# kmacrow/Shellac

Measured on AMD Instinct MI355X. Metric: cache_ops_per_s, higher is better.
Workload: dtype uint8

## Files before the change

### shellac_amd/csrc/bind.cc

```cpp
#include <pybind11/pybind11.h>
#include <pybind11/stl.h>

#include <hip/hip_runtime_api.h>

#include "bind_parts.h"
#include "hbm_cache.h"
#include "host_cache.h"
#include "trace.h"

namespace py = pybind11;
using namespace shellac;

namespace {

template <typename T>
T* P(uintptr_t p) { return reinterpret_cast<T*>(p); }
hipStream_t S(uintptr_t s) { return reinterpret_cast<hipStream_t>(s); }

py::dict counters_dict(const CacheCounters& c) {
  py::dict d;
  d["get_ops"] = c.get_ops;
  d["get_hits"] = c.get_hits;
  d["get_bytes"] = c.get_bytes;
  d["set_ops"] = c.set_ops;
// ... 93 lines not shown
         py::arg("now"), py::arg("stream"), py::arg("done_slot") = -1)
      .def("serve_get", [](HbmCache& c, uintptr_t host_keys, int64_t n, uintptr_t out,
                           uint64_t out_cap, uintptr_t off, uint32_t now, int done_slot,
                           uintptr_t stream) {
        py::gil_scoped_release nogil;
        return c.serve_get_after(S(stream), P<const Digest>(host_keys), n, P<uint8_t>(out),
                                 out_cap, P<uint64_t>(off), now, done_slot);
      }, py::arg("host_keys"), py::arg("n"), py::arg("out"), py::arg("out_cap"), py::arg("off"),
         py::arg("now"), py::arg("done_slot"), py::arg("stream") = 0)
      .def("serve_wait", [](HbmCache& c, int slot, int64_t timeout_ms) {
        py::gil_scoped_release nogil;
        return c.serve_wait(slot, timeout_ms);
      }, py::arg("slot"), py::arg("timeout_ms") = 10000)
      .def("serve_kick", [](HbmCache& c) {
        py::gil_scoped_release nogil;
        c.serve_kick();
      })
      .def("serve_stop", [](HbmCache& c) {
        py::gil_scoped_release nogil;
        c.serve_stop();
      })
      .def("serve_trace", &HbmCache::serve_trace)
      .def_property_readonly("wall_khz", &HbmCache::wall_khz)
      .def_property_readonly("serve_launches", &HbmCache::serve_launches)
      .def_property_readonly("serve_jobs", &HbmCache::serve_jobs)
      .def("host_slot", &HbmCache::host_slot)
      .def("wait_host_slot", [](const HbmCache& c, int i, int64_t timeout_ms) {
        py::gil_scoped_release nogil;
        return c.wait_host_slot(i, timeout_ms);
      }, py::arg("slot"), py::arg("timeout_ms") = 10000)
      .def("gather", [](HbmCache& c, uintptr_t loc, uintptr_t off, int64_t n, uintptr_t out,
                        uintptr_t s, uint64_t out_cap, uintptr_t first, uintptr_t size,
                        uintptr_t out_size, uintptr_t out_off, uintptr_t table, uintptr_t cslot,
                        uintptr_t prefix, int shift) {
        py::gil_scoped_release nogil;
        c.gather(P<const uint64_t>(loc), P<const uint64_t>(off), n, P<uint8_t>(out), S(s),
                 out_cap, P<const uint32_t>(first), P<const uint64_t>(size), P<uint64_t>(out_size),
                 P<uint64_t>(out_off), P<uint32_t>(table), P<const uint32_t>(cslot),
                 P<const uint64_t>(prefix), shift);
      }, py::arg("loc"), py::arg("off"), py::arg("n"), py::arg("out"), py::arg("stream"),
         py::arg("out_cap") = ~0ull, py::arg("first") = 0, py::arg("size") = 0,
         py::arg("out_size") = 0, py::arg("out_off") = 0, py::arg("table") = 0,
         py::arg("cslot") = 0, py::arg("prefix") = 0, py::arg("shift") = 0)
      .def("store_graph", [](HbmCache& c, HbmCache::StoreGraph& g, uintptr_t keys,
                             uintptr_t values, uintptr_t val_off, uintptr_t vlen, uintptr_t flags,
                             uintptr_t expire, int64_t n, uint64_t bytes_bound, uint32_t now,
                             uintptr_t s) {
        py::gil_scoped_release nogil;
        c.store_graph(&g, P<const Digest>(keys), P<const uint8_t>(values),
                      P<const uint64_t>(val_off), P<const uint32_t>(vlen),
                      P<const uint32_t>(flags), P<const uint32_t>(expire), n, bytes_bound, now,
                      S(s));
      })
      .def("store", [](HbmCache& c, uintptr_t keys, uintptr_t values, uintptr_t val_off,
                       uintptr_t vlen, uintptr_t flags, uintptr_t expire, int64_t n,
                       uint64_t bytes_bound, uint32_t now, uintptr_t s, uintptr_t index_after,
                       uintptr_t append_after, uintptr_t append_done, int phase,
                       uintptr_t plan_done, uintptr_t done) {
        py::gil_scoped_release nogil;
        c.store(P<const Digest>(keys), P<const uint8_t>(values), P<const uint64_t>(val_off),
                P<const uint32_t>(vlen), P<const uint32_t>(flags), P<const uint32_t>(expire), n,
                bytes_bound, now, S(s), reinterpret_cast<hipEvent_t>(index_after), true,
                reinterpret_cast<hipEvent_t>(append_after),
                reinterpret_cast<hipEvent_t>(append_done), phase,
                reinterpret_cast<hipEvent_t>(plan_done), reinterpret_cast<hipEvent_t>(done));
      }, py::arg("keys"), py::arg("values"), py::arg("val_off"), py::arg("vlen"),
         py::arg("flags"), py::arg("expire"), py::arg("n"), py::arg("bytes_bound"), py::arg("now"),
         py::arg("stream"), py::arg("index_after") = 0, py::arg("append_after") = 0,
         py::arg("append_done") = 0, py::arg("phase") = 0, py::arg("plan_done") = 0,
         py::arg("done") = 0)
      .def("remove", [](HbmCache& c, uintptr_t keys, int64_t n, uintptr_t found, uint32_t now,
                        uintptr_t s) {
        py::gil_scoped_release nogil;
        c.remove(P<const Digest>(keys), n, P<uint8_t>(found), now, S(s));
      })
      .def("sweep", [](HbmCache& c, uint32_t now, uintptr_t s) {
// ... 239 lines not shown
```

### shellac_amd/csrc/hbm_cache.h

```cpp
#pragma once

#include <hip/hip_runtime_api.h>

#include <algorithm>
#include <mutex>
#include <string>
#include <vector>

#include "layout.h"

namespace shellac {

enum : int { kEvictFifo = 0, kEvictClock = 1 };

struct ShardConfig {
  uint64_t log_bytes = 1ull << 30;
  uint64_t nbuckets = 1ull << 20;
  uint32_t max_item = 1u << 20;
  int device = 0;
  int evict = kEvictClock;
  uint64_t reinsert_max = 0;
  int serve_blocks = 8;
};

// ... 23 lines not shown
  static constexpr uint64_t kSlotFailed = ~0ull - 1;
  static constexpr int64_t kLookupPrefixWords = 2049;
  void small_get(const Digest* keys, int64_t n, uint8_t* out, uint64_t out_cap, uint64_t* off,
                 uint32_t now, hipStream_t s, int done_slot = -1);
  static constexpr int64_t kSmallGetMax = 1 << 17;
  static constexpr int kServeKeys = 29;
  static constexpr int kServeRing = 16;
  bool serve_get(const Digest* host_keys, int64_t n, uint8_t* out, uint64_t out_cap,
                 uint64_t* off, uint32_t now, int done_slot);
  bool serve_get_after(hipStream_t after, const Digest* host_keys, int64_t n, uint8_t* out,
                       uint64_t out_cap, uint64_t* off, uint32_t now, int done_slot);
  void serve_kick();
  uint64_t serve_backlog() const {
    uint64_t c = 0;
    for (int b = 0; b < srv_blocks_; ++b)
      c += __atomic_load_n(srv_ctl_ + kSrvCtlConsumed + 8 * b, __ATOMIC_ACQUIRE);
    const uint64_t t = __atomic_load_n(&srv_ticket_, __ATOMIC_RELAXED);
    return t > c ? t - c : 0;
  }
  static constexpr int kServeBlocksMax = 8;
  static constexpr int kSrvCtlConsumed = 24;
  int serve_blocks() const { return srv_blocks_; }
  uint64_t serve_wait(int done_slot, int64_t timeout_ms = 10000);
  void serve_stop();
  uint64_t serve_launches() const { return srv_launches_; }
  uint64_t serve_jobs() const { return __atomic_load_n(&srv_ticket_, __ATOMIC_RELAXED); }
  std::vector<uint64_t> serve_trace() const;
  uint64_t wall_khz() const { return srv_khz_; }
  void gather(const uint64_t* loc, const uint64_t* off, int64_t n, uint8_t* out, hipStream_t s,
              uint64_t out_cap = ~0ull, const uint32_t* first = nullptr,
              const uint64_t* size = nullptr, uint64_t* out_size = nullptr,
              uint64_t* out_off = nullptr, uint32_t* table = nullptr,
              const uint32_t* cslot = nullptr, const uint64_t* prefix = nullptr,
              int shift = 0);
  void store(const Digest* keys, const uint8_t* values, const uint64_t* val_off,
             const uint32_t* vlen, const uint32_t* flags, const uint32_t* expire, int64_t n,
             uint64_t bytes_bound, uint32_t now, hipStream_t s, hipEvent_t index_after = nullptr,
             bool allow_reclaim = true, hipEvent_t append_after = nullptr,
             hipEvent_t append_done = nullptr, int phase = 0, hipEvent_t plan_done = nullptr,
             hipEvent_t done = nullptr);
  bool would_reclaim(uint64_t bytes_bound) const {
    return cfg_.evict == kEvictClock && rmax_ && should_reclaim(bytes_bound);
  }
  struct StoreGraph {
    hipGraphExec_t exec[2] = {nullptr, nullptr};
    const void* ptrs[6] = {};
    int64_t n = -1;
    uint64_t bound = 0;
    uint32_t now = 0;
    uint64_t ws_gen = 0;
    uint64_t captures = 0, launches = 0;
  };
  void store_graph(StoreGraph* g, const Digest* keys, const uint8_t* values,
                   const uint64_t* val_off, const uint32_t* vlen, const uint32_t* flags,
                   const uint32_t* expire, int64_t n, uint64_t bytes_bound, uint32_t now,
                   hipStream_t s);
  static void destroy_graph(StoreGraph* g);
  void remove(const Digest* keys, int64_t n, uint8_t* found, uint32_t now, hipStream_t s);
  void sweep(uint32_t now, hipStream_t s, uint64_t* live_entries, uint64_t* live_bytes);
  uint64_t export_keys(Digest* out, uint64_t out_cap, uint32_t now, hipStream_t s);
  void save(const std::string& path, const uint64_t user[4], hipStream_t s);
  void load(const std::string& path, uint64_t user[4], hipStream_t s);
  void flush(hipStream_t s);
  std::vector<uint64_t> debug_bucket(uint64_t b);
  std::vector<uint64_t> debug_hand();
  void debug_set_entry(uint64_t b, int slot, uint64_t d0, uint64_t d1, uint64_t loc,
                       uint32_t vlen, uint32_t expire);
// ... 188 lines not shown
```

### shellac_amd/csrc/hbm_cache.hip

```cpp
#include <hip/hip_runtime.h>
#include <hip/hip_ext.h>
#include <hipcub/hipcub.hpp>

#include <algorithm>
#include <chrono>
#include <cstdlib>
#include <cstring>
#include <type_traits>
#include <vector>

#include "hbm_cache.h"
#include "trace.h"

namespace shellac {

#define HIP_OK(expr)                                                                   \
  do {                                                                                 \
    hipError_t _e = (expr);                                                            \
    if (_e != hipSuccess)                                                              \
      throw Error(std::string("HIP error ") + hipGetErrorString(_e) + " at " + #expr + \
                  " [" + __FILE__ + ":" + std::to_string(__LINE__) + "]");             \
  } while (0)

namespace {
// ... 364 lines not shown
        int he;
        uint64_t hb = bucket1(d, mask);
        group_match(vb[p], d, l8, head, cap, now, &hl, &hv, &he);
        if (hl == 0) {
          hb = bucket2(d, mask);
          const uint4 v2 = reinterpret_cast<const uint4*>(index + hb * kEntriesPerBucket)[l8];
          group_match(v2, d, l8, head, cap, now, &hl, &hv, &he);
        }
        if (l8 == 0) {
          ++ops;
          if (hl) {
            mark_ref(index, hb, he, hv);
            hv = entry_vlen(hv);
            out_loc[i] = (hl - 1) % cap;
            out_size[i] = item_bytes(hv);
            ++hits;
            bytes += hv;
            psum += item_bytes(hv);
          } else {
            out_loc[i] = kMissLoc;
            out_size[i] = 0;
          }
        }
      }
    }
    __syncthreads();
  }
  block_count(ctr, ops, &CacheCounters::get_ops, hits, &CacheCounters::get_hits, bytes,
              &CacheCounters::get_bytes);
  block_partial(psum, part);
}

constexpr int kCoPer = 4;
constexpr int kCoKeys = kBlock * kCoPer;
constexpr int kCoSlots = 2 * kCoKeys;

template <bool PROBE>
__global__ __launch_bounds__(kBlock) __attribute__((amdgpu_waves_per_eu(4))) void k_coalesce(
    const Digest* __restrict__ keys, int64_t n, int64_t plen, uint32_t* __restrict__ tab,
    uint32_t tmask, uint32_t* __restrict__ first, uint32_t* __restrict__ cslot,
    Entry* __restrict__ index, uint64_t mask, const uint64_t* __restrict__ head_ptr,
    uint64_t reserve, uint64_t cap, uint32_t now, uint64_t* __restrict__ out_loc,
    uint64_t* __restrict__ out_size, CacheCounters* __restrict__ ctr,
    uint64_t* __restrict__ part, int local_only, uint64_t* __restrict__ woff) {
  __shared__ Digest s_k[kCoKeys];
  __shared__ unsigned long long s_wt[kBlock / 64], s_run;
  if (threadIdx.x == 0) s_run = 0;
  __shared__ uint32_t s_tab[kCoSlots];
  __shared__ uint32_t s_rep[kCoKeys];
  __shared__ uint32_t s_dup[kCoKeys];
  __shared__ uint32_t s_q[PROBE ? kCoKeys : 1];
  __shared__ int s_qn;
  const uint64_t head = PROBE ? *head_ptr + reserve : 0;
  const int l8 = threadIdx.x & 7;
  unsigned long long ops = 0, hits = 0, bytes = 0, psum = 0, dups = 0;
  const int64_t r0 = (int64_t)blockIdx.x * plen, r1 = min(n, r0 + plen);
  for (int64_t base = r0; base < r1; base += kCoKeys) {
    const int cnt = (int)min((int64_t)kCoKeys, r1 - base);
    for (int k = threadIdx.x; k < kCoSlots; k += kBlock) s_tab[k] = 0;
    for (int k = threadIdx.x; k < kCoKeys; k += kBlock) s_dup[k] = 0;
    if (threadIdx.x == 0) s_qn = 0;
    Digest dk[kCoPer];
    uint32_t lrep[kCoPer];
#pragma unroll
    for (int u = 0; u < kCoPer; ++u) {
      const int j = u * kBlock + threadIdx.x;
      lrep[u] = (uint32_t)j;
      if (j < cnt) {
        dk[u] = keys[base + j];
        s_k[j] = dk[u];
      }
    }
    __syncthreads();
#pragma unroll
    for (int u = 0; u < kCoPer; ++u) {
      const int j = u * kBlock + threadIdx.x;
      if (j >= cnt) continue;
// ... 68 lines not shown
    if (PROBE) {
      const int qn = s_qn;
      constexpr int kG = kBlock / 8;
      for (int q0 = threadIdx.x >> 3; q0 < qn; q0 += kG * kCoProbe) {
        uint4 vb[kCoProbe];
#pragma unroll
        for (int p = 0; p < kCoProbe; ++p) {
          const int q = q0 + p * kG;
          if (q < qn)
            vb[p] = reinterpret_cast<const uint4*>(
                index + bucket1(s_k[s_q[q]], mask) * kEntriesPerBucket)[l8];
        }
#pragma unroll
        for (int p = 0; p < kCoProbe; ++p) {
          const int q = q0 + p * kG;
          if (q >= qn) continue;
          const int j = (int)s_q[q];
          const Digest d = s_k[j];
          uint64_t hl;
          uint32_t hv;
          int he;
          uint64_t hb = bucket1(d, mask);
          group_match(vb[p], d, l8, head, cap, now, &hl, &hv, &he);
          if (hl == 0) {
            hb = bucket2(d, mask);
            const uint4 v2 = reinterpret_cast<const uint4*>(index + hb * kEntriesPerBucket)[l8];
            group_match(v2, d, l8, head, cap, now, &hl, &hv, &he);
          }
          if (l8 == 0) {
            if (hl) mark_ref(index, hb, he, hv);
            hv = entry_vlen(hv);
            ++ops;
            out_loc[base + j] = hl ? (hl - 1) % cap : kMissLoc;
            out_size[base + j] = hl ? item_bytes(hv) : 0;
            if (woff) s_tab[j] = hl ? (uint32_t)item_bytes(hv) : 0u;
            if (hl) {
              ++hits;
              bytes += hv;
              psum += item_bytes(hv);
            }
          }
        }
      }
    }
#pragma unroll
    for (int u = 0; u < kCoPer; ++u) {
      const int j = u * kBlock + threadIdx.x;
      if (j >= cnt) continue;
      const uint32_t f = s_rep[lrep[u]];
      first[base + j] = f;
      if (PROBE && f != (uint32_t)(base + j)) {
        out_loc[base + j] = kMissLoc;
        out_size[base + j] = 0;
        if (woff) s_tab[j] = 0u;
        ++dups;
      }
    }
    __syncthreads();
    if (PROBE && woff) {
      const int t4 = threadIdx.x * kCoPer;
      uint32_t v[kCoPer];
      unsigned long long ts = 0;
#pragma unroll
      for (int u = 0; u < kCoPer; ++u) {
        v[u] = t4 + u < cnt ? s_tab[t4 + u] : 0u;
        ts += v[u];
      }
      const int lane = threadIdx.x & 63, wv = threadIdx.x >> 6;
      unsigned long long inc = ts;
#pragma unroll
      for (int d = 1; d < 64; d <<= 1) {
        const unsigned long long o = __shfl_up(inc, d);
        if (lane >= d) inc += o;
      }
      if (lane == 63) s_wt[wv] = inc;
      __syncthreads();
      unsigned long long ex = s_run + inc - ts, tot = 0;
#pragma unroll
      for (int k = 0; k < kBlock / 64; ++k) {
        if (k < wv) ex += s_wt[k];
        tot += s_wt[k];
      }
#pragma unroll
      for (int u = 0; u < kCoPer; ++u) {
        if (t4 + u < cnt) woff[base + t4 + u] = ex;
        ex += v[u];
      }
      __syncthreads();
      if (threadIdx.x == 0) s_run += tot;
    }
  }
  if (PROBE) {
    if (blockIdx.x == 0 && threadIdx.x == 0) out_size[n] = 0;
    block_count(ctr, ops, &CacheCounters::get_ops, hits, &CacheCounters::get_hits, bytes,
                &CacheCounters::get_bytes);
    block_count(ctr, dups, &CacheCounters::get_coalesced);
    block_partial(psum, part);
  }
}

static_assert(HbmCache::kLookupPrefixWords == kMaxGrid + 1, "prefix words: kMaxGrid + 1");
__global__ __launch_bounds__(kBlock) void k_block_prefix(const uint64_t* __restrict__ part,
                                                         int nparts,
                                                         uint64_t* __restrict__ prefix,
                                                         uint64_t* __restrict__ host_total) {
  constexpr int kPer = kMaxGrid / kBlock;
  __shared__ unsigned long long s_w[kBlock / 64];
  const int lane = threadIdx.x & 63, w = threadIdx.x >> 6;
  uint64_t v[kPer];
  unsigned long long ts = 0;
#pragma unroll
  for (int u = 0; u < kPer; ++u) {
    const int i = threadIdx.x * kPer + u;
    v[u] = i < nparts ? part[i] : 0;
    ts += v[u];
  }
  unsigned long long inc = ts;
#pragma unroll
  for (int d = 1; d < 64; d <<= 1) {
    const unsigned long long o = __shfl_up(inc, d);
    if (lane >= d) inc += o;
  }
  if (lane == 63) s_w[w] = inc;
  __syncthreads();
  unsigned long long ex = inc - ts;
  for (int k = 0; k < w; ++k) ex += s_w[k];
// ... 33 lines not shown
                                                       const uint32_t* __restrict__ cslot) {
  for (int64_t i = (int64_t)blockIdx.x * kBlock + threadIdx.x; i < n;
       i += (int64_t)gridDim.x * kBlock) {
    const uint32_t f = first[i];
    out_size[i] = size[f];
    out_off[i] = off[f];
    if (f == (uint32_t)i && tab) tab[cslot[i]] = 0u;
  }
}

template <typename T>
__device__ __forceinline__ int64_t seg_search(const T* off, int64_t lo, int64_t hi, uint64_t x) {
  while (hi - lo > 1) {
    const int64_t mid = (lo + hi) >> 1;
    if ((uint64_t)off[mid] <= x) lo = mid; else hi = mid;
  }
  return lo;
}

__device__ __forceinline__ int64_t seg_search_global(const uint64_t* off, int64_t n, uint64_t x) {
  int64_t lo = 0, hi = n;
  while (hi - lo > 1) {
    const int64_t mid = (lo + hi) >> 1;
    if (off[mid] <= x) lo = mid; else hi = mid;
  }
  return lo;
}

struct PlainOff {
  const uint64_t* __restrict__ p;
  __device__ __forceinline__ uint64_t operator[](int64_t j) const { return p[j]; }
};
struct BlockedOff {
  const uint64_t* __restrict__ local;
  const uint64_t* __restrict__ prefix;
  int64_t n;
  int shift;
  __device__ __forceinline__ uint64_t operator[](int64_t j) const {
    return j < n ? prefix[j >> shift] + local[j] : prefix[((n - 1) >> shift) + 1];
  }
};

template <typename Off>
__device__ __forceinline__ void block_find2(const Off off, int64_t n1,
                                            uint64_t x0, uint64_t x1, int64_t* s_lo,
                                            int64_t* s_hi, int* s_cnt) {
  const int h = threadIdx.x >> 7, t = threadIdx.x & 127, w = threadIdx.x >> 6;
  const uint64_t x = h ? x1 : x0;
  if (threadIdx.x < 2) {
    s_lo[threadIdx.x] = 0;
    s_hi[threadIdx.x] = n1;
  }
  __syncthreads();
  for (int round = 0; round < 16; ++round) {
    const int64_t lo = s_lo[h], hi = s_hi[h];
    const bool done = (s_hi[0] - s_lo[0] <= 1) && (s_hi[1] - s_lo[1] <= 1);
    if (done) break;
    const int64_t len = hi - lo;
    bool ok = false;
    if (len > 1 && t < 127) {
      const int64_t p = lo + (len * (t + 1) + 127) / 128;
      ok = p < hi && off[p] <= x;
    }
    const unsigned long long b = __ballot(ok);
    __syncthreads();
    if ((threadIdx.x & 63) == 0) s_cnt[w] = __popcll(b);
    __syncthreads();
    if (t == 0 && len > 1) {
      const int k = s_cnt[2 * h] + s_cnt[2 * h + 1];
      const int64_t nlo = k > 0 ? lo + (len * k + 127) / 128 : lo;
      const int64_t nhi = k < 127 ? lo + (len * (k + 1) + 127) / 128 : hi;
      s_lo[h] = nlo;
// ... 27 lines not shown
    if (threadIdx.x < kBlock - 1) {
      const int64_t q = l + (len * (threadIdx.x + 1) + kBlock - 1) / kBlock;
      ok = q < h && off[q] <= x;
    }
    const unsigned long long b = __ballot(ok);
    __syncthreads();
    if ((threadIdx.x & 63) == 0) s_cnt[threadIdx.x >> 6] = __popcll(b);
    __syncthreads();
    if (threadIdx.x == 0) {
      int k = 0;
#pragma unroll
      for (int w = 0; w < kBlock / 64; ++w) k += s_cnt[w];
      const int64_t nlo = k > 0 ? l + (len * k + kBlock - 1) / kBlock : l;
      const int64_t nhi = k < kBlock - 1 ? l + (len * (k + 1) + kBlock - 1) / kBlock : h;
      s_b[0] = nlo;
      s_b[1] = nhi < h ? nhi : h;
    }
    __syncthreads();
  }
  return s_b[0];
}

struct ExpandTail {
  const uint32_t* first = nullptr;
  int64_t n = 0;
  const uint64_t* size = nullptr;
  const uint64_t* off = nullptr;
  uint64_t* out_size = nullptr;
  uint64_t* out_off = nullptr;
  uint32_t* tab = nullptr;
  const uint32_t* cslot = nullptr;
  const uint64_t* prefix = nullptr;
  int shift = 0;
};
__device__ __forceinline__ void expand_tail(const ExpandTail& ex) {
  for (int64_t i = (int64_t)blockIdx.x * kBlock + threadIdx.x; i < ex.n;
       i += (int64_t)gridDim.x * kBlock) {
    const uint32_t f = ex.first[i];
    ex.out_size[i] = ex.size[f];
    ex.out_off[i] = ex.prefix ? ex.prefix[f >> ex.shift] + ex.off[f] : ex.off[f];
    if (f == (uint32_t)i && ex.tab) ex.tab[ex.cslot[i]] = 0u;
  }
}

template <int MODE, int U, int WAVES, bool NTSTORE = false, bool GLDS = false>
__global__ __launch_bounds__(kBlock) __attribute__((amdgpu_waves_per_eu(WAVES))) void k_segcopy(
    const uint8_t* __restrict__ src, const uint64_t* __restrict__ src_off,
    const uint64_t* __restrict__ dst_off, int64_t n, uint8_t* __restrict__ dst,
    const Digest* __restrict__ keys, const uint32_t* __restrict__ vlen,
    const uint32_t* __restrict__ flags, const uint32_t* __restrict__ expire,
    const uint64_t* __restrict__ head_ptr, uint64_t cap, int min_tile, ExpandTail ex) {
  do {
  constexpr int TSC = MODE == 2 ? 768 : GLDS ? 512 : kTileSegCap;
  __shared__ uint64_t s_off[TSC + 1];
  __shared__ __attribute__((aligned(16))) uint8_t s_stage[GLDS ? kBlock / 64 : 1][GLDS ? U : 1]
                                                         [GLDS ? 1024 : 16];
  __shared__ uint64_t s_src[TSC];
  __shared__ int64_t s_lo[2], s_hi[2];
  __shared__ int s_cnt[kBlock / 64];
  if (MODE == 3) n = *reinterpret_cast<const int64_t*>(head_ptr);
  using Off = typename std::conditional<MODE == 4, BlockedOff, PlainOff>::type;
  Off doff;
  if constexpr (MODE == 4)
    doff = BlockedOff{dst_off, ex.prefix, n, ex.shift};
  else
    doff = PlainOff{dst_off};
  const uint64_t total = doff[n];
  if ((MODE == 0 || MODE == 3 || MODE == 4) && total > cap) break;
  const uint64_t* __restrict__ seg_len = MODE == 2 ? head_ptr : nullptr;
  __shared__ uint32_t s_len[MODE == 2 ? TSC : 1];
  const int64_t nchunks = (int64_t)(total >> 4);
  const uint64_t base = MODE == 1 ? *head_ptr % cap : 0;
  (void)s_len;
  int64_t span = (nchunks + gridDim.x - 1) / gridDim.x;
  span = (span + kBlock - 1) & ~(int64_t)(kBlock - 1);
  if (span < min_tile) span = min_tile;
  const int64_t r0 = (int64_t)blockIdx.x * span;
  const int64_t r1 = min(r0 + span, nchunks);
  if (r0 >= r1) break;
  block_find2(doff, n + 1, (uint64_t)r0 << 4, ((uint64_t)r1 << 4) - 1, s_lo, s_hi, s_cnt);
  const int64_t ja = uniform64(s_lo[0]), jb = uniform64(s_lo[1]);
  for (int64_t j0 = ja; j0 <= jb; j0 += TSC) {
    if (j0 > ja && j0 < jb) {
      const uint64_t o0 = doff[j0];
      if (doff[j0 + 1] == o0) j0 = uniform64(block_last_le(doff, j0, jb + 1, o0, s_lo, s_cnt));
    }
    const int cnt = (int)min((int64_t)TSC, jb - j0 + 1);
    __syncthreads();
    for (int k = threadIdx.x; k <= cnt; k += kBlock) s_off[k] = doff[j0 + k];
    for (int k = threadIdx.x; k < cnt; k += kBlock) s_src[k] = src_off[j0 + k];
    if (MODE == 2)
      for (int k = threadIdx.x; k < cnt; k += kBlock) {
        const uint64_t st = dst_off[j0 + k], ln = seg_len[j0 + k];
        s_len[k] = st + ln <= cap ? (uint32_t)ln : 0u;
      }
    __syncthreads();
    const int64_t c0 = max(r0, (int64_t)(s_off[0] >> 4));
    const int64_t c1 = min(r1, (int64_t)(s_off[cnt] >> 4));
    int jl = 0;
    const int64_t nu = (c1 - c0 + kBlock - 1) / kBlock;
#pragma unroll 1
    for (int64_t u0 = 0; u0 < nu; u0 += U) {
      const u32x4* sp[U];
      u32x4 v[U];
      uint64_t dofs[MODE == 1 ? U : 1];
#pragma unroll
      for (int u = 0; u < U; ++u) {
        const int64_t c = c0 + (u0 + u) * kBlock + threadIdx.x;
        sp[u] = nullptr;
        if (c >= c1) continue;
        const uint64_t x = (uint64_t)c << 4;
        int step = 1, hi;
        while (jl + step < cnt && s_off[jl + step] <= x) {
          jl += step;
          step <<= 1;
        }
        hi = min(jl + step, cnt);
        while (hi - jl > 1) {
          const int mid = (jl + hi) >> 1;
          if (s_off[mid] <= x) jl = mid; else hi = mid;
        }
        const uint64_t seg_start = s_off[jl];
        const uint64_t seg_src = s_src[jl];
// ... 2071 lines not shown
  HIP_OK(hipGetLastError());
  launch_offsets(size, n, part_, grid, off, s, ht);
}

void HbmCache::lookup_slots(const Digest* keys, int64_t nslots, int64_t slot_rows,
                            const int64_t* slot_cnt, uint64_t* loc, uint64_t* size, uint64_t* off,
                            uint32_t now, hipStream_t s, const uint64_t* reserve_dev) {
  TraceRange tr("hbm.lookup_slots");
  std::lock_guard<std::mutex> lk(mu_);
  DeviceGuard g(cfg_.device);
  const int64_t n = nslots * slot_rows;
  if (n <= 0) {
    HIP_OK(hipMemsetAsync(off, 0, sizeof(uint64_t), s));
    return;
  }
  const int grid = grid_for(n * 8, kBlock, kMaxGrid);
  hipLaunchKernelGGL(k_probe, dim3(grid), dim3(kBlock), 0, s, keys, n, index_, cfg_.nbuckets - 1,
                     cur_head(), (uint64_t)0, cfg_.log_bytes, now, loc, size, ctr_, part_,
                     (const uint32_t*)nullptr, slot_rows, slot_cnt, reserve_dev);
  HIP_OK(hipGetLastError());
  launch_offsets(size, n, part_, grid, off, s, nullptr);
}

int HbmCache::lookup_coalesced(const Digest* keys, int64_t n, uint32_t* table,
                               int64_t table_slots, uint32_t* first, uint64_t* loc,
                               uint64_t* size, uint64_t* off, uint32_t now, hipStream_t s,
                               uint64_t reserve, int total_slot, uint32_t* cslot,
                               bool table_clean, uint64_t* prefix, hipEvent_t index_done) {
  TraceRange tr("hbm.lookup_coalesced");
  SH_CHECK(total_slot < kHostSlots, "host slot out of range");
  SH_CHECK(n < (1ll << 31), "coalesce: batch too large");
  SH_CHECK(table_slots >= 2 * n && (table_slots & (table_slots - 1)) == 0,
           "coalesce: table needs a power of two >= 2n slots");
  std::lock_guard<std::mutex> lk(mu_);
  DeviceGuard g(cfg_.device);
  uint64_t* ht = total_slot >= 0 ? host_slots_ + total_slot : nullptr;
  if (ht) __atomic_store_n(ht, kSlotPending, __ATOMIC_RELEASE);
  if (n <= 0) {
    HIP_OK(hipMemsetAsync(off, 0, sizeof(uint64_t), s));
    if (prefix) HIP_OK(hipMemsetAsync(prefix, 0, sizeof(uint64_t), s));
    if (ht) *ht = 0;
    if (index_done) HIP_OK(hipEventRecord(index_done, s));
    return prefix ? 31 : -1;
  }
  if (!table_clean) HIP_OK(hipMemsetAsync(table, 0, (size_t)table_slots * sizeof(uint32_t), s));
  const int64_t chunks = (n + kCoKeys - 1) / kCoKeys;
  int64_t per = (chunks + kMaxGrid - 1) / kMaxGrid;
  if (prefix)
    for (int64_t p2 = 1;; p2 <<= 1)
      if (p2 >= per) {
        per = p2;
        break;
      }
  const int grid = (int)((chunks + per - 1) / per);
  const int64_t plen = per * kCoKeys;
  launch_stop(&index_done, k_coalesce<true>, dim3(grid), dim3(kBlock), s, keys, n, plen, table,
              (uint32_t)(table_slots - 1), first, cslot, index_, cfg_.nbuckets - 1, cur_head(),
              reserve, cfg_.log_bytes, now, loc, size, ctr_, part_, 0, prefix ? off : nullptr);
  HIP_OK(hipGetLastError());
  if (!prefix) {
    launch_offsets(size, n, part_, grid, off, s, ht, plen);
    return -1;
  }
  hipLaunchKernelGGL(k_block_prefix, dim3(1), dim3(kBlock), 0, s, part_, grid, prefix, ht);
  HIP_OK(hipGetLastError());
  int shift = 0;
// ... 132 lines not shown
  std::vector<uint64_t> out(srv_trace_, srv_trace_ + kSrvTrace * 8);
  return out;
}

uint64_t HbmCache::serve_wait(int i, int64_t timeout_ms) {
  SH_CHECK(i >= 0 && i < kHostSlots, "host slot out of range");
  const auto t0 = std::chrono::steady_clock::now();
  for (uint32_t spin = 0;; ++spin) {
    const uint64_t v = __atomic_load_n(host_slots_ + i, __ATOMIC_ACQUIRE);
    if (v != kSlotPending) return v;
    if ((spin & 255) == 255) {
      serve_kick();
      const auto el = std::chrono::steady_clock::now() - t0;
      SH_CHECK(std::chrono::duration_cast<std::chrono::milliseconds>(el).count() < timeout_ms,
               "timed out waiting for the edge server");
    }
    __builtin_ia32_pause();
  }
}

void HbmCache::serve_stop() {
  std::lock_guard<std::mutex> lk(srv_mu_);
  if (!srv_running_) return;
  DeviceGuard g(cfg_.device);
  __atomic_store_n(srv_ctl_ + kCtlStop, 1ull, __ATOMIC_RELEASE);
  HIP_OK(hipStreamSynchronize(srv_stream_));
  srv_running_ = false;
}

void HbmCache::gather(const uint64_t* loc, const uint64_t* off, int64_t n, uint8_t* out,
                      hipStream_t s, uint64_t out_cap, const uint32_t* first,
                      const uint64_t* size, uint64_t* out_size, uint64_t* out_off,
                      uint32_t* table, const uint32_t* cslot, const uint64_t* prefix,
                      int shift) {
  TraceRange tr("hbm.gather");
  DeviceGuard g(cfg_.device);
  if (n <= 0) return;
  ExpandTail ex;
  if (first) ex = ExpandTail{first, n, size, off, out_size, out_off, table, cslot};
  ex.prefix = prefix;
  ex.shift = shift;
  if (prefix)
    launch_segcopy_ex<4>(s, ex, log_, loc, off, n, out, nullptr, nullptr, nullptr, nullptr,
                         nullptr, out_cap);
  else
    launch_segcopy_ex<0>(s, ex, log_, loc, off, n, out, nullptr, nullptr, nullptr, nullptr,
                         nullptr, out_cap);
  HIP_OK(hipGetLastError());
}

void HbmCache::store(const Digest* keys, const uint8_t* values, const uint64_t* val_off,
                     const uint32_t* vlen, const uint32_t* flags, const uint32_t* expire,
                     int64_t n, uint64_t bytes_bound, uint32_t now, hipStream_t s,
                     hipEvent_t index_after, bool allow_reclaim, hipEvent_t append_after,
                     hipEvent_t append_done, int phase, hipEvent_t plan_done,
                     hipEvent_t done) {
  TraceRange tr("hbm.store");
  if (n <= 0) {
    if (done) HIP_OK(hipEventRecord(done, s));
    return;
  }
  SH_CHECK(bytes_bound <= cfg_.log_bytes / 2,
           "SET batch larger than half the log; split the batch");
  std::lock_guard<std::mutex> lk(mu_);
  DeviceGuard g(cfg_.device);
  note_stream(s);
  stop_ev_ = done;
  struct EndMark {
    HbmCache* c;
    hipStream_t s;
    ~EndMark() {
      if (c->stop_ev_) {
        (void)hipEventRecord(c->stop_ev_, s);
        c->stop_ev_ = nullptr;
// ... 408 lines not shown
```

### shellac_amd/ops/cache.py

```python
from __future__ import annotations

import time
from dataclasses import dataclass
from typing import Iterable, Optional, Sequence

import numpy as np
import torch

from .._native import core

ITEM_HEADER_BYTES = 32
ITEM_MAGIC = 0x5348A11C
MISS_LOC = (1 << 64) - 1


def _stream_handle(device: torch.device) -> int:
    return torch.cuda.current_stream(device).cuda_stream


def item_bytes(vlen: int) -> int:
    return ITEM_HEADER_BYTES + ((vlen + 15) & ~15)


def pack_bytes(items: Sequence[bytes]) -> tuple[np.ndarray, np.ndarray]:
# ... 126 lines not shown

    def elapsed_time(self, end: "StreamEvent") -> float:
        return float(core().event_elapsed_ms(self.handle, end.handle))

    def __del__(self):
        h = getattr(self, "handle", 0)
        if h:
            try:
                core().event_destroy(h)
            except Exception:
                pass


def _event_handle(ev) -> int:
    if ev is None:
        return 0
    if isinstance(ev, StreamEvent):
        return ev.handle
    return ev.cuda_event



def _stop_handle(ev) -> int:
    if ev is None:
        return 0
    if not isinstance(ev, StreamEvent):
        raise TypeError("a stop event must be a StreamEvent")
    return ev.handle


@dataclass
class Lookup:
    loc: torch.Tensor
    size: torch.Tensor
    off_raw: torch.Tensor
    prefix: Optional[torch.Tensor] = None
    shift: int = 0

    @property
    def off(self) -> torch.Tensor:
        if self.prefix is not None:
            raise ValueError("a blocked lookup holds workgroup-local offsets: the per-request "
                             "offsets come from the gather's expand tail")
        return self.off_raw

    @property
    def n(self) -> int:
        return self.loc.numel()

    def total(self) -> torch.Tensor:
        if self.prefix is None:
            return self.off_raw[self.n:self.n + 1]
        nb = ((self.n - 1) >> self.shift) + 1 if self.n else 0
        return self.prefix[nb:nb + 1]

    def hits(self) -> torch.Tensor:
        return self.size[: self.n] > 0


def reserve_step_streams(device) -> None:
    dev = torch.device(device)
    if dev.type == "cuda":
        core().step_streams(dev.index if dev.index is not None else torch.cuda.current_device())


class CacheShard:

# ... 43 lines not shown
    def lookup(self, keys: torch.Tensor, now: Optional[int] = None,
               reserve_bytes: int = 0, total_slot: int = -1,
               first: Optional[torch.Tensor] = None) -> Lookup:
        self._check(keys, "keys")
        n = keys.shape[0]
        loc = torch.empty(n, dtype=torch.int64, device=self.device)
        size = torch.empty(n + 1, dtype=torch.int64, device=self.device)
        off = torch.empty(n + 1, dtype=torch.int64, device=self.device)
        now = self.now() if now is None else now
        if self.is_gpu:
            if first is not None:
                self._check(first, "first")
                if first.numel() != n or first.dtype != torch.int32:
                    raise ValueError("first must be int32 [n] from coalesce()")
            self._impl.lookup(keys.data_ptr(), n, loc.data_ptr(), size.data_ptr(), off.data_ptr(),
                              now, self._s(), int(reserve_bytes), int(total_slot),
                              first.data_ptr() if first is not None else 0)
        else:
            size[n] = 0
            self._impl.lookup(keys.data_ptr(), n, loc.data_ptr(), size.data_ptr(), off.data_ptr(),
                              now, int(reserve_bytes))
        return Lookup(loc, size, off)

    def lookup_coalesced(self, keys: torch.Tensor, now: Optional[int] = None,
                         reserve_bytes: int = 0, total_slot: int = -1,
                         table: Optional[torch.Tensor] = None, blocked: bool = False,
                         index_done=None):
        if not self.is_gpu or keys.shape[0] == 0:
            return self.lookup(keys, now, reserve_bytes, total_slot), None, None
        self._check(keys, "keys")
        c = core()
        n = keys.shape[0]
        cslot = None
        if table is None:
            slots = int(c.coalesce_table_slots(n))
            table = torch.empty(slots, dtype=torch.int32, device=self.device)
        else:
            slots = table.numel()
            if slots < int(c.coalesce_table_slots(n)) or slots & (slots - 1):
                raise ValueError("coalescing table too small or not a power of two")
            cslot = torch.empty(n, dtype=torch.int32, device=self.device)
        first = torch.empty(n, dtype=torch.int32, device=self.device)
        loc = torch.empty(n, dtype=torch.int64, device=self.device)
        size = torch.empty(n + 1, dtype=torch.int64, device=self.device)
        off = torch.empty(n + 1, dtype=torch.int64, device=self.device)
        now = self.now() if now is None else now
        prefix = (torch.empty(int(c.LOOKUP_PREFIX_WORDS), dtype=torch.int64, device=self.device)
                  if blocked else None)
        shift = self._impl.lookup_coalesced(keys.data_ptr(), n, table.data_ptr(), slots,
                                            first.data_ptr(), loc.data_ptr(), size.data_ptr(),
                                            off.data_ptr(), now, self._s(), int(reserve_bytes),
                                            int(total_slot),
                                            cslot.data_ptr() if cslot is not None else 0,
                                            cslot is not None,
                                            prefix.data_ptr() if prefix is not None else 0,
                                            _stop_handle(index_done))
        return Lookup(loc, size, off, prefix, max(int(shift), 0)), first, cslot

    def host_total(self, slot: int, timeout_ms: int = 10000) -> int:
        return int(self._impl.wait_host_slot(slot, timeout_ms))

    def small_get(self, keys: torch.Tensor, out_cap: int = 16 << 20,
                  now: Optional[int] = None, done_slot: int = -1):
        assert self.is_gpu and keys.shape[0] <= int(core().SMALL_GET_MAX)
        self._check(keys, "keys")
        n = keys.shape[0]
        out = torch.empty(max(int(out_cap), 16), dtype=torch.uint8, device=self.device)
        off = torch.empty(n + 1, dtype=torch.int64, device=self.device)
        self._impl.small_get(keys.data_ptr(), n, out.data_ptr(), int(out_cap), off.data_ptr(),
                             self.now() if now is None else now, self._s(), int(done_slot))
        return out, off

    def serve_get(self, keys: torch.Tensor, out_cap: int = 16 << 20,
                  now: Optional[int] = None, done_slot: int = 5, timeout_ms: int = 10000):
        assert self.is_gpu
        keys = keys.to("cpu").contiguous()
        n = keys.shape[0]
        out = torch.zeros(max(int(out_cap), 16), dtype=torch.uint8, device=self.device)
        off = torch.zeros(n + 1, dtype=torch.int64, device=self.device)
        if not self._impl.serve_get(keys.data_ptr(), n, out.data_ptr(), int(out_cap),
                                    off.data_ptr(), self.now() if now is None else now,
                                    int(done_slot), self._s()):
            return None
        self._impl.serve_wait(int(done_slot), int(timeout_ms))
        return out, off

    def gather(self, lk: Lookup, out: Optional[torch.Tensor] = None,
               total: Optional[int] = None, out_cap: Optional[int] = None,
               expand=None) -> torch.Tensor:
        if out is None:
            total = int(lk.total().item()) if total is None else total
            out = torch.empty(max(total, 16), dtype=torch.uint8, device=self.device)
        self._check(out, "out")
        if self.is_gpu:
            cap = out.numel() if out_cap is None else min(int(out_cap), out.numel())
            ex = [0] * 6
            if expand is not None:
                first, osz, ooff, table, cslot = expand
                ex = [first.data_ptr(), lk.size.data_ptr(), osz.data_ptr(), ooff.data_ptr(),
                      table.data_ptr() if table is not None else 0,
                      cslot.data_ptr() if cslot is not None else 0]
            elif lk.prefix is not None:
                raise ValueError("a blocked lookup's offsets are read only with an expand tail")
            self._impl.gather(lk.loc.data_ptr(), lk.off_raw.data_ptr(), lk.n, out.data_ptr(),
                              self._s(), cap, *ex,
                              lk.prefix.data_ptr() if lk.prefix is not None else 0, lk.shift)
        else:
            self._impl.gather(lk.loc.data_ptr(), lk.off.data_ptr(), lk.n, out.data_ptr())
        return out

    def get(self, keys: torch.Tensor, now: Optional[int] = None):
        if not self.is_gpu:
            lk = self.lookup(keys, now)
            return self.gather(lk), lk.off[: lk.n], lk.size[: lk.n]
        lk = self.lookup(keys, now, total_slot=1)
        out = self.gather(lk, total=self.host_total(1))
        return out, lk.off[: lk.n], lk.size[: lk.n]

    @staticmethod
    def payload_bound(n: int, payload_bytes: int) -> int:
        return 48 * int(n) + int(payload_bytes)

    def set_bound(self, n: int, payload_bytes: int) -> int:
        return self.payload_bound(n, payload_bytes) + int(self._impl.reinsert_max)

    def store(self, keys: torch.Tensor, values: torch.Tensor, val_off: torch.Tensor,
              vlen: torch.Tensor, flags: Optional[torch.Tensor] = None,
              expire: Optional[torch.Tensor] = None, now: Optional[int] = None,
              bytes_bound: Optional[int] = None,
              index_after=None, append_after=None, append_done=None, phase: int = 0,
              plan_done=None, done=None) -> None:
        for t, nm in ((keys, "keys"), (values, "values"), (val_off, "val_off"), (vlen, "vlen")):
            self._check(t, nm)
        if vlen.dtype != torch.int32 or val_off.dtype != torch.int64:
            raise TypeError("vlen must be int32 and val_off int64")
        n = keys.shape[0]
        if n == 0:
            if done is not None and self.is_gpu:
                done.record(torch.cuda.current_stream(self.device))
# ... 87 lines not shown
```

Before: 3.343 billion.

## Pack per-row size and local offset into one word for blocked lookups

In the blocked (prefix) lookup path, the probe kernel now writes one 64-bit word per row holding the local offset and the item size, instead of separate size and offset arrays. Gather and the expand tail unpack that word, and the expand tail now clears the coalescing table wholesale with vector stores rather than scattering zeros through cslot, so the cslot buffer is no longer allocated. This is meant to cut global memory writes and reads in lookup and gather. The cost is size-limit checks on max_item and an alignment requirement on the table.

```diff
diff --git a/shellac_amd/csrc/bind.cc b/shellac_amd/csrc/bind.cc
--- a/shellac_amd/csrc/bind.cc
+++ b/shellac_amd/csrc/bind.cc
@@ -149,16 +149,17 @@
       .def("gather", [](HbmCache& c, uintptr_t loc, uintptr_t off, int64_t n, uintptr_t out,
                         uintptr_t s, uint64_t out_cap, uintptr_t first, uintptr_t size,
                         uintptr_t out_size, uintptr_t out_off, uintptr_t table, uintptr_t cslot,
-                        uintptr_t prefix, int shift) {
+                        uintptr_t prefix, int shift, int64_t table_slots) {
         py::gil_scoped_release nogil;
         c.gather(P<const uint64_t>(loc), P<const uint64_t>(off), n, P<uint8_t>(out), S(s),
                  out_cap, P<const uint32_t>(first), P<const uint64_t>(size), P<uint64_t>(out_size),
                  P<uint64_t>(out_off), P<uint32_t>(table), P<const uint32_t>(cslot),
-                 P<const uint64_t>(prefix), shift);
+                 P<const uint64_t>(prefix), shift, table_slots);
       }, py::arg("loc"), py::arg("off"), py::arg("n"), py::arg("out"), py::arg("stream"),
          py::arg("out_cap") = ~0ull, py::arg("first") = 0, py::arg("size") = 0,
          py::arg("out_size") = 0, py::arg("out_off") = 0, py::arg("table") = 0,
-         py::arg("cslot") = 0, py::arg("prefix") = 0, py::arg("shift") = 0)
+         py::arg("cslot") = 0, py::arg("prefix") = 0, py::arg("shift") = 0,
+         py::arg("table_slots") = 0)
       .def("store_graph", [](HbmCache& c, HbmCache::StoreGraph& g, uintptr_t keys,
                              uintptr_t values, uintptr_t val_off, uintptr_t vlen, uintptr_t flags,
                              uintptr_t expire, int64_t n, uint64_t bytes_bound, uint32_t now,
diff --git a/shellac_amd/csrc/hbm_cache.h b/shellac_amd/csrc/hbm_cache.h
--- a/shellac_amd/csrc/hbm_cache.h
+++ b/shellac_amd/csrc/hbm_cache.h
@@ -79,7 +79,7 @@
               const uint64_t* size = nullptr, uint64_t* out_size = nullptr,
               uint64_t* out_off = nullptr, uint32_t* table = nullptr,
               const uint32_t* cslot = nullptr, const uint64_t* prefix = nullptr,
-              int shift = 0);
+              int shift = 0, int64_t table_slots = 0);
   void store(const Digest* keys, const uint8_t* values, const uint64_t* val_off,
              const uint32_t* vlen, const uint32_t* flags, const uint32_t* expire, int64_t n,
              uint64_t bytes_bound, uint32_t now, hipStream_t s, hipEvent_t index_after = nullptr,
diff --git a/shellac_amd/csrc/hbm_cache.hip b/shellac_amd/csrc/hbm_cache.hip
--- a/shellac_amd/csrc/hbm_cache.hip
+++ b/shellac_amd/csrc/hbm_cache.hip
@@ -420,6 +420,11 @@
 }
 
 constexpr int kCoPer = 4;
+constexpr int kPackBits = 21;
+constexpr uint64_t kPackSizeMask = (1ull << kPackBits) - 1;
+__device__ __forceinline__ uint64_t pack_row(uint64_t local_off, uint32_t bytes) {
+  return local_off << kPackBits | bytes;
+}
 constexpr int kCoKeys = kBlock * kCoPer;
 constexpr int kCoSlots = 2 * kCoKeys;
 
@@ -430,7 +435,7 @@
     Entry* __restrict__ index, uint64_t mask, const uint64_t* __restrict__ head_ptr,
     uint64_t reserve, uint64_t cap, uint32_t now, uint64_t* __restrict__ out_loc,
     uint64_t* __restrict__ out_size, CacheCounters* __restrict__ ctr,
-    uint64_t* __restrict__ part, int local_only, uint64_t* __restrict__ woff) {
+    uint64_t* __restrict__ part, int local_only, uint64_t* __restrict__ packed) {
   __shared__ Digest s_k[kCoKeys];
   __shared__ unsigned long long s_wt[kBlock / 64], s_run;
   if (threadIdx.x == 0) s_run = 0;
@@ -565,8 +570,10 @@
             hv = entry_vlen(hv);
             ++ops;
             out_loc[base + j] = hl ? (hl - 1) % cap : kMissLoc;
-            out_size[base + j] = hl ? item_bytes(hv) : 0;
-            if (woff) s_tab[j] = hl ? (uint32_t)item_bytes(hv) : 0u;
+            if (packed)
+              s_tab[j] = hl ? (uint32_t)item_bytes(hv) : 0u;
+            else
+              out_size[base + j] = hl ? item_bytes(hv) : 0;
             if (hl) {
               ++hits;
               bytes += hv;
@@ -583,14 +590,17 @@
       const uint32_t f = s_rep[lrep[u]];
       first[base + j] = f;
       if (PROBE && f != (uint32_t)(base + j)) {
-        out_loc[base + j] = kMissLoc;
-        out_size[base + j] = 0;
-        if (woff) s_tab[j] = 0u;
+        if (packed) {
+          s_tab[j] = 0u;
+        } else {
+          out_loc[base + j] = kMissLoc;
+          out_size[base + j] = 0;
+        }
         ++dups;
       }
     }
     __syncthreads();
-    if (PROBE && woff) {
+    if (PROBE && packed) {
       const int t4 = threadIdx.x * kCoPer;
       uint32_t v[kCoPer];
       unsigned long long ts = 0;
@@ -616,7 +626,7 @@
       }
 #pragma unroll
       for (int u = 0; u < kCoPer; ++u) {
-        if (t4 + u < cnt) woff[base + t4 + u] = ex;
+        if (t4 + u < cnt) packed[base + t4 + u] = pack_row(ex, v[u]);
         ex += v[u];
       }
       __syncthreads();
@@ -624,7 +634,7 @@
     }
   }
   if (PROBE) {
-    if (blockIdx.x == 0 && threadIdx.x == 0) out_size[n] = 0;
+    if (!packed && blockIdx.x == 0 && threadIdx.x == 0) out_size[n] = 0;
     block_count(ctr, ops, &CacheCounters::get_ops, hits, &CacheCounters::get_hits, bytes,
                 &CacheCounters::get_bytes);
     block_count(ctr, dups, &CacheCounters::get_coalesced);
@@ -724,12 +734,13 @@
   __device__ __forceinline__ uint64_t operator[](int64_t j) const { return p[j]; }
 };
 struct BlockedOff {
-  const uint64_t* __restrict__ local;
+  const uint64_t* __restrict__ packed;
   const uint64_t* __restrict__ prefix;
   int64_t n;
   int shift;
   __device__ __forceinline__ uint64_t operator[](int64_t j) const {
-    return j < n ? prefix[j >> shift] + local[j] : prefix[((n - 1) >> shift) + 1];
+    return j < n ? prefix[j >> shift] + (packed[j] >> kPackBits)
+                 : prefix[((n - 1) >> shift) + 1];
   }
 };
 
@@ -823,13 +834,53 @@
   const uint32_t* cslot = nullptr;
   const uint64_t* prefix = nullptr;
   int shift = 0;
+  int64_t tab_words = 0;
 };
+__device__ __forceinline__ void expand_tail_packed(const ExpandTail& ex) {
+  constexpr int kRows = 4;
+  const int64_t stride = (int64_t)gridDim.x * kBlock;
+  for (int64_t i0 = (int64_t)blockIdx.x * kBlock + threadIdx.x; i0 < ex.n;
+       i0 += kRows * stride) {
+    uint32_t f[kRows];
+    uint64_t p[kRows], pre[kRows];
+#pragma unroll
+    for (int u = 0; u < kRows; ++u) {
+      const int64_t i = i0 + u * stride;
+      f[u] = i < ex.n ? ex.first[i] : 0u;
+    }
+#pragma unroll
+    for (int u = 0; u < kRows; ++u) {
+      p[u] = ex.off[f[u]];
+      pre[u] = ex.prefix[f[u] >> ex.shift];
+    }
+#pragma unroll
+    for (int u = 0; u < kRows; ++u) {
+      const int64_t i = i0 + u * stride;
+      if (i >= ex.n) continue;
+      ex.out_size[i] = p[u] & kPackSizeMask;
+      ex.out_off[i] = pre[u] + (p[u] >> kPackBits);
+    }
+  }
+  if (ex.tab) {
+    const int64_t n4 = ex.tab_words >> 2;
+    u32x4* __restrict__ t4 = reinterpret_cast<u32x4*>(ex.tab);
+    for (int64_t k = (int64_t)blockIdx.x * kBlock + threadIdx.x; k < n4; k += stride)
+      t4[k] = u32x4{0u, 0u, 0u, 0u};
+    if (blockIdx.x == 0 && threadIdx.x < (ex.tab_words & 3))
+      ex.tab[(n4 << 2) + threadIdx.x] = 0u;
+  }
+}
+
 __device__ __forceinline__ void expand_tail(const ExpandTail& ex) {
+  if (ex.prefix) {
+    expand_tail_packed(ex);
+    return;
+  }
   for (int64_t i = (int64_t)blockIdx.x * kBlock + threadIdx.x; i < ex.n;
        i += (int64_t)gridDim.x * kBlock) {
     const uint32_t f = ex.first[i];
     ex.out_size[i] = ex.size[f];
-    ex.out_off[i] = ex.prefix ? ex.prefix[f >> ex.shift] + ex.off[f] : ex.off[f];
+    ex.out_off[i] = ex.off[f];
     if (f == (uint32_t)i && ex.tab) ex.tab[ex.cslot[i]] = 0u;
   }
 }
@@ -878,8 +929,22 @@
     }
     const int cnt = (int)min((int64_t)TSC, jb - j0 + 1);
     __syncthreads();
-    for (int k = threadIdx.x; k <= cnt; k += kBlock) s_off[k] = doff[j0 + k];
-    for (int k = threadIdx.x; k < cnt; k += kBlock) s_src[k] = src_off[j0 + k];
+    if constexpr (MODE == 4) {
+      for (int k = threadIdx.x; k <= cnt; k += kBlock) {
+        const int64_t j = j0 + k;
+        if (j < n) {
+          const uint64_t p = dst_off[j];
+          s_off[k] = ex.prefix[j >> ex.shift] + (p >> kPackBits);
+          if (k < cnt) s_src[k] = (p & kPackSizeMask) ? src_off[j] : kSegSkip;
+        } else {
+          s_off[k] = total;
+          if (k < cnt) s_src[k] = kSegSkip;
+        }
+      }
+    } else {
+      for (int k = threadIdx.x; k <= cnt; k += kBlock) s_off[k] = doff[j0 + k];
+      for (int k = threadIdx.x; k < cnt; k += kBlock) s_src[k] = src_off[j0 + k];
+    }
     if (MODE == 2)
       for (int k = threadIdx.x; k < cnt; k += kBlock) {
         const uint64_t st = dst_off[j0 + k], ln = seg_len[j0 + k];
@@ -3017,6 +3082,10 @@
   SH_CHECK(n < (1ll << 31), "coalesce: batch too large");
   SH_CHECK(table_slots >= 2 * n && (table_slots & (table_slots - 1)) == 0,
            "coalesce: table needs a power of two >= 2n slots");
+  static_assert(kMaxGrid == 2048 && 20 + kPackBits <= 64 - kPackBits,
+                "packed rows: a workgroup's local offsets must fit 64 - kPackBits bits");
+  SH_CHECK(!prefix || item_bytes(cfg_.max_item) <= kPackSizeMask,
+           "blocked lookup: a record of max_item bytes does not fit a packed row");
   std::lock_guard<std::mutex> lk(mu_);
   DeviceGuard g(cfg_.device);
   uint64_t* ht = total_slot >= 0 ? host_slots_ + total_slot : nullptr;
@@ -3215,7 +3284,7 @@
                       hipStream_t s, uint64_t out_cap, const uint32_t* first,
                       const uint64_t* size, uint64_t* out_size, uint64_t* out_off,
                       uint32_t* table, const uint32_t* cslot, const uint64_t* prefix,
-                      int shift) {
+                      int shift, int64_t table_slots) {
   TraceRange tr("hbm.gather");
   DeviceGuard g(cfg_.device);
   if (n <= 0) return;
@@ -3223,6 +3292,11 @@
   if (first) ex = ExpandTail{first, n, size, off, out_size, out_off, table, cslot};
   ex.prefix = prefix;
   ex.shift = shift;
+  if (prefix && first && table) {
+    SH_CHECK(table_slots > 0 && ((uintptr_t)table & 15) == 0,
+             "gather: a blocked lookup's table is cleared whole (16-byte aligned, its slots)");
+    ex.tab_words = table_slots;
+  }
   if (prefix)
     launch_segcopy_ex<4>(s, ex, log_, loc, off, n, out, nullptr, nullptr, nullptr, nullptr,
                          nullptr, out_cap);
diff --git a/shellac_amd/ops/cache.py b/shellac_amd/ops/cache.py
--- a/shellac_amd/ops/cache.py
+++ b/shellac_amd/ops/cache.py
@@ -182,7 +182,7 @@
 @dataclass
 class Lookup:
     loc: torch.Tensor
-    size: torch.Tensor
+    size: Optional[torch.Tensor]
     off_raw: torch.Tensor
     prefix: Optional[torch.Tensor] = None
     shift: int = 0
@@ -292,6 +292,7 @@
         c = core()
         n = keys.shape[0]
         cslot = None
+        table_clean = False
         if table is None:
             slots = int(c.coalesce_table_slots(n))
             table = torch.empty(slots, dtype=torch.int32, device=self.device)
@@ -299,20 +300,23 @@
             slots = table.numel()
             if slots < int(c.coalesce_table_slots(n)) or slots & (slots - 1):
                 raise ValueError("coalescing table too small or not a power of two")
-            cslot = torch.empty(n, dtype=torch.int32, device=self.device)
+            table_clean = True
+            if not blocked:
+                cslot = torch.empty(n, dtype=torch.int32, device=self.device)
         first = torch.empty(n, dtype=torch.int32, device=self.device)
         loc = torch.empty(n, dtype=torch.int64, device=self.device)
-        size = torch.empty(n + 1, dtype=torch.int64, device=self.device)
+        size = None if blocked else torch.empty(n + 1, dtype=torch.int64, device=self.device)
         off = torch.empty(n + 1, dtype=torch.int64, device=self.device)
         now = self.now() if now is None else now
         prefix = (torch.empty(int(c.LOOKUP_PREFIX_WORDS), dtype=torch.int64, device=self.device)
                   if blocked else None)
         shift = self._impl.lookup_coalesced(keys.data_ptr(), n, table.data_ptr(), slots,
-                                            first.data_ptr(), loc.data_ptr(), size.data_ptr(),
+                                            first.data_ptr(), loc.data_ptr(),
+                                            size.data_ptr() if size is not None else 0,
                                             off.data_ptr(), now, self._s(), int(reserve_bytes),
                                             int(total_slot),
                                             cslot.data_ptr() if cslot is not None else 0,
-                                            cslot is not None,
+                                            table_clean,
                                             prefix.data_ptr() if prefix is not None else 0,
                                             _stop_handle(index_done))
         return Lookup(loc, size, off, prefix, max(int(shift), 0)), first, cslot
@@ -354,17 +358,20 @@
         self._check(out, "out")
         if self.is_gpu:
             cap = out.numel() if out_cap is None else min(int(out_cap), out.numel())
-            ex = [0] * 6
+            ex, slots = [0] * 6, 0
             if expand is not None:
                 first, osz, ooff, table, cslot = expand
-                ex = [first.data_ptr(), lk.size.data_ptr(), osz.data_ptr(), ooff.data_ptr(),
+                ex = [first.data_ptr(), lk.size.data_ptr() if lk.size is not None else 0,
+                      osz.data_ptr(), ooff.data_ptr(),
                       table.data_ptr() if table is not None else 0,
                       cslot.data_ptr() if cslot is not None else 0]
+                slots = table.numel() if table is not None else 0
             elif lk.prefix is not None:
                 raise ValueError("a blocked lookup's offsets are read only with an expand tail")
             self._impl.gather(lk.loc.data_ptr(), lk.off_raw.data_ptr(), lk.n, out.data_ptr(),
                               self._s(), cap, *ex,
-                              lk.prefix.data_ptr() if lk.prefix is not None else 0, lk.shift)
+                              lk.prefix.data_ptr() if lk.prefix is not None else 0, lk.shift,
+                              slots)
         else:
             self._impl.gather(lk.loc.data_ptr(), lk.off.data_ptr(), lk.n, out.data_ptr())
         return out
```

Result: faster. 3.510 billion (median of 6 runs) (+5.0%).
